# AKASH2907/pi-consistency-activity-detection

Hardware: AMD Instinct MI355X
Metric: train clips/sec (bs=8, 16×224×224, I3D+caps+bv cons) at 1/2/4/8 GPU (higher is better)
Workload: dtype f32 (fp32 operands and fp32 accumulation everywhere; 33 of the 79 conv / input-gradient launches and the 3x3x3 / 1x1x1 weight gradients multiply on the bf16 matrix cores: every fp32 operand as the exact sum of 3 bf16 terms, 6 products on v_mfma_f32_32x32x16_bf16, hi / lo fp32 accumulators -- error v

## Files before the change

### include/picons.h

```cpp
#ifndef PICONS_H
#define PICONS_H
#include <stdint.h>
#ifdef __cplusplus
extern "C" {
#endif

typedef void* pc_stream;

#define PC_OK            0
#define PC_E_ARG        -1
#define PC_E_LAUNCH     -2
#define PC_E_NODEVICE   -3

#define PC_ACT_NONE 0
#define PC_ACT_RELU 1
#define PC_ACT_SIGMOID 2

#define PC_F_ACCUM   1
#define PC_F_BIAS    2
#define PC_F_CSCALE  4
#define PC_F_BNPART  8
#define PC_F_NFAST   16
#define PC_F_TOUT    32
#define PC_F_CI3     64
// ... 109 lines not shown
int pc_bn_eval_stat(const float* gamma, const float* beta, const float* running_mean,
                    const float* running_var, float eps, int C, float* stat, pc_stream s);
int64_t pc_bn_bwd_ws_floats(int64_t rows, int C, int groups);
int pc_bn_bwd(const float* dy, int lddy, const float* z, int ldz, const float* stat, int C,
              int64_t rows, int groups, int relu, float* dz, int lddz, float* dgamma, float* dbeta,
              int accum, float* ws, pc_stream s);

typedef struct pc_pool_desc {
    int32_t N, Ti, Hi, Wi, C, ldi;
    int32_t To, Ho, Wo, ldo;
    int32_t k[3], s[3], padf[3];
} pc_pool_desc;
int pc_maxpool_fwd(const pc_pool_desc* d, const float* x, float* y, uint8_t* argmax, pc_stream s);
int pc_maxpool_bwd(const pc_pool_desc* d, const float* dy, const uint8_t* argmax, float* dx,
                   int accum, pc_stream s);

int pc_channel_scale(const float* x, int ldx, const float* scale, int N, int64_t pos_per_n, int C,
                     float* y, int ldy, int accum, pc_stream s);
int64_t pc_act_bwd_ws_floats(int64_t rows, int C);
int pc_act_bwd(const float* dy, int lddy, const float* y, int ldy, int act, int C, int64_t rows,
               float* dz, int lddz, float* dbias, int accum, float* ws, pc_stream s);
int pc_ncdhw_to_ndhwc(const void* src, int src_is_f64, int N, int C, int64_t thw, int W, int Cpad,
                      int flipw, float* dst, pc_stream s);
int pc_ndhwc_to_ncdhw(const float* src, int ld, int N, int C, int64_t thw, float* dst, pc_stream s);
int pc_transpose_batched(const float* src, int batch, int R, int Cc, int64_t src_batch_stride,
                         int src_ld, float* dst, int64_t dst_batch_stride, int dst_ld, int accum,
                         pc_stream s);
typedef struct pc_transpose_job {
    uint64_t src, dst;
    int64_t  src_batch_stride, dst_batch_stride;
// ... 208 lines not shown
```

### pi-consistency-activity-detection_amd/capi.py

```python
import ctypes as C
import os

import numpy as np

_HERE = os.path.dirname(os.path.abspath(__file__))
DIAG = os.environ.get("PICONS_DIAG_LIB", "0") not in ("", "0")
DIAG_SWITCHES = ("PICONS_CONV_ABLATE", "PICONS_WGRAD_ABLATE", "PICONS_WINO_VARIANT")
LIB_PATH = os.path.join(_HERE, "libpicons_diag.so" if DIAG else "libpicons.so")
if os.environ.get("PICONS_LIB_NAME"):
    LIB_PATH = os.path.join(_HERE, os.path.basename(os.environ["PICONS_LIB_NAME"]))
_lib = None

i32, i64, f32, vp = C.c_int32, C.c_int64, C.c_float, C.c_void_p


class ConvDesc(C.Structure):
    _fields_ = [(n, i32) for n in ("N", "Ti", "Hi", "Wi", "Ci", "ldi", "Tq", "Hq", "Wq", "To", "Ho", "Wo", "Co", "ldo")] + \
               [(n, i32 * 3) for n in ("ostr", "ooff", "istr", "ntap", "ioff0", "istep", "wk0", "wkstep")] + \
               [(n, i32) for n in ("KT", "KH", "KW", "ldw", "act", "flags", "wgstride", "bgstride", "act_c0", "groups")]


class WgradDesc(C.Structure):
    _fields_ = [(n, i32) for n in ("N", "Tq", "Hq", "Wq", "Cd", "ldd", "Ts", "Hs", "Ws", "Cs", "lds")] + \
               [(n, i32 * 3) for n in ("istr", "ntap", "ioff0", "istep", "wk0")] + [(n, i32) for n in ("KT", "KH", "KW", "splitk", "nbatch", "dbstride", "sbstride", "gbstride", "Td", "Hd", "Wd")] + [("doff", i32 * 3), ("flags", i32), ("ws_slices", i32)]
# ... 16 lines not shown


class LossDesc(C.Structure):
    _fields_ = [(n, i32) for n in ("B", "T", "H", "W", "bv", "gv", "n_frames", "predict_maps", "jhmdb")] + \
               [(n, f32) for n in ("lower_thresh", "upper_thresh", "bv_wt", "gv_wt", "wt_loc", "wt_cons", "wt_ramp")]


OP_DTYPE = np.dtype([("kind", np.int32), ("i", np.int32, 48), ("f", np.float32, 8), ("lane", np.int32),
                     ("p", np.uint64, 12), ("l", np.int64, 4)], align=False)

(OP_CONV, OP_WGRAD, OP_BN_FINALIZE, OP_BN_APPLY, OP_BN_EVAL_STAT, OP_BN_BWD, OP_POOL_FWD, OP_POOL_BWD, OP_CHSCALE,
 OP_ACT_BWD, OP_TO_NDHWC, OP_TO_NCDHW, OP_TRANSPOSE, OP_FILL, OP_AXPY, OP_EM_FWD, OP_EM_BWD, OP_CMASK_FWD, OP_CMASK_BWD,
 OP_TAPSUM_FWD, OP_TAPSUM_BWD, OP_LOSS, OP_SPREAD, OP_ADAM, OP_TAIL_COMBINE, OP_TAIL_COLSUM, OP_TAIL_GRADS, OP_COL2IM,
 OP_AXIS, OP_WSPEC_FWD, OP_WSPEC_BWD, OP_WSPEC_MASTER_FWD, OP_WSPEC_MASTER_BWD, OP_TAIL6_WEIGHTS, OP_TAIL6_GATHER, OP_TAIL6_SCATTER, OP_TAIL6_WGRAD_MAP, OP_TAIL6_BIAS_SUMS,
 OP_TRANSPOSE_MULTI, OP_FORK, OP_JOIN, OP_WGRAD_MULTI, OP_WINO_CONV, OP_WINO_WEIGHTS, OP_CONV_X6, OP_SPLIT_PLANES, OP_SPLIT_PLANES_MULTI, OP_WSPEC_MASTER_PLANES, OP_BN_FIN_APPLY, OP_WGRAD_FOLD, OP_WINO_WEIGHTS_MULTI, OP_VAL_METRICS) = range(1, 53)
MAX_LANES = 8

WJOB_DTYPE = np.dtype([("d", np.int32, 42), ("D", np.uint64), ("S", np.uint64), ("g", np.uint64)], align=False)

TJOB_DTYPE = np.dtype([("src", np.uint64), ("dst", np.uint64), ("sbs", np.int64), ("dbs", np.int64), ("batch", np.int32), ("R", np.int32),
                       ("C", np.int32), ("sld", np.int32), ("dld", np.int32), ("accum", np.int32), ("nslices", np.int32), ("reserved", np.int32),
                       ("sst", np.int64)], align=False)

SJOB_DTYPE = np.dtype([("src", np.uint64), ("planes", np.uint64), ("n", np.int64), ("pstride", np.int64)], align=False)

WWJOB_DTYPE = np.dtype([("w", np.uint64), ("U", np.uint64), ("sO", np.int64), ("sT", np.int64), ("sI", np.int64), ("O", np.int32), ("I", np.int32),
                        ("KT", np.int32), ("flip", np.int32), ("m", np.int32), ("reserved", np.int32)], align=False)

ACT_NONE, ACT_RELU, ACT_SIGMOID = 0, 1, 2
F_ACCUM, F_BIAS, F_CSCALE, F_BNPART, F_NFAST, F_TOUT, F_CI3, F_X6, F_STRIPS = 1, 2, 4, 8, 16, 32, 64, 128, 256
# ... 31 lines not shown
    "pc_wino4_u_floats": (i64, [i32, i32, i32]),
    "pc_wino4_weights": (i32, [vp, i64, i64, i64, i32, i32, i32, i32, vp, vp]),
    "pc_wino_bnpart_rows": (i32, [C.POINTER(WinoDesc)]),
    "pc_wino_work": (i32, [C.POINTER(WinoDesc), C.POINTER(C.c_double)]),
    "pc_bn_finalize": (i32, [vp, i32, i32, i32, i64, vp, vp, f32, f32, vp, vp, vp, vp]),
    "pc_bn_finalize_ws": (i32, [vp, i32, i32, i32, i64, vp, vp, f32, f32, vp, vp, vp, vp, vp]),
    "pc_bn_finalize_ws_floats": (i64, [i32, i32, i32]),
    "pc_bn_finalize_apply_ok": (i32, [i32, i32]),
    "pc_bn_finalize_apply": (i32, [vp, i32, i32, i32, i64, vp, vp, f32, f32, vp, vp, vp, vp, i32, i64, vp, i32, i32, vp]),
    "pc_bn_apply": (i32, [vp, i32, vp, i32, i64, i32, vp, i32, i32, vp]),
    "pc_bn_eval_stat": (i32, [vp, vp, vp, vp, f32, i32, vp, vp]),
    "pc_bn_bwd_ws_floats": (i64, [i64, i32, i32]),
    "pc_bn_bwd": (i32, [vp, i32, vp, i32, vp, i32, i64, i32, i32, vp, i32, vp, vp, i32, vp, vp]),
    "pc_maxpool_fwd": (i32, [C.POINTER(PoolDesc), vp, vp, vp, vp]),
    "pc_maxpool_bwd": (i32, [C.POINTER(PoolDesc), vp, vp, vp, i32, vp]),
    "pc_channel_scale": (i32, [vp, i32, vp, i32, i64, i32, vp, i32, i32, vp]),
    "pc_act_bwd_ws_floats": (i64, [i64, i32]),
    "pc_act_bwd": (i32, [vp, i32, vp, i32, i32, i32, i64, vp, i32, vp, i32, vp, vp]),
    "pc_ncdhw_to_ndhwc": (i32, [vp, i32, i32, i32, i64, i32, i32, i32, vp, vp]),
    "pc_ndhwc_to_ncdhw": (i32, [vp, i32, i32, i32, i64, vp, vp]),
    "pc_transpose_batched": (i32, [vp, i32, i32, i32, i64, i32, vp, i64, i32, i32, vp]),
    "pc_col2im": (i32, [vp, i32, i32, i32, i32, i32, i32, vp, i32, i32, vp]),
    "pc_seg_frame_counts": (i32, [vp, vp, i64, i64, vp, vp]),
    "pc_map_accumulate": (i32, [vp, i64, i32, i32, vp, vp, vp, vp, vp]),
    "pc_val_record_words": (i32, [i32]),
    "pc_val_metrics_ws_floats": (i64, [i32, i64]),
    "pc_val_metrics": (i32, [vp, vp, vp, vp, i32, i64, i32, vp, vp, vp]),
    "pc_clip_from_u8": (i32, [vp, i32, i32, i32, C.POINTER(C.c_int32), i32, i32, i32, vp, i32, vp, vp, vp, vp]),
    "pc_clip_from_u8_ndhwc4": (i32, [vp, i32, i32, i32, C.POINTER(C.c_int32), i32, i32, i32, vp, i32, vp, vp, vp, vp]),
    "pc_clip_from_u8_masks": (i32, [vp, i32, i32, i32, C.POINTER(C.c_int32), i32, i32, i32, vp, C.POINTER(C.c_int32), vp, vp, vp, vp, vp]),
# ... 122 lines not shown
```

### pi-consistency-activity-detection_amd/csrc/api.hip

```cpp
#include "common.h"
#include <string.h>
#include <vector>

static thread_local char g_err[512] = "";

void pc_set_error(const char* fmt, ...) {
    va_list ap;
    va_start(ap, fmt);
    vsnprintf(g_err, sizeof(g_err), fmt, ap);
    va_end(ap);
}

extern "C" const char* pc_last_error(void) { return g_err; }
extern "C" int pc_version(void) { return PC_VERSION; }

extern "C" int pc_transpose_batched(const float*, int, int, int, int64_t, int, float*, int64_t, int, int, pc_stream);

#define P(T, k) ((T)(uintptr_t)op.p[k])

static int run_one(const pc_op& op, pc_stream s) {
    switch (op.kind) {
        case PC_OP_CONV: {
            pc_conv_desc d;
            memcpy(&d, op.i, sizeof(d));
// ... 8 lines not shown
            return pc_split_planes(P(const float*, 0), P(uint16_t*, 1), op.l[0], op.l[1], s);
        case PC_OP_WSPEC_MASTER_PLANES:
            return pc_wspec_master_planes(P(const float*, 0), P(const float*, 1), op.i[0], op.i[1], op.i[2], op.i[3], op.i[4], op.i[5], op.i[6], op.i[7],
                                          P(uint16_t*, 2), P(uint16_t*, 3), op.l[0], s);
        case PC_OP_SPLIT_PLANES_MULTI:
            return pc_split_planes_multi(P(const pc_split_job*, 0), op.i[0], s);
        case PC_OP_WGRAD: {
            pc_wgrad_desc d;
            memcpy(&d, op.i, sizeof(d));
            return pc_conv_wgrad(&d, P(const float*, 0), P(const float*, 1), P(float*, 2), s);
        }
        case PC_OP_BN_FINALIZE:
            return pc_bn_finalize_ws(P(const float*, 0), op.i[0], op.i[1], op.i[2], op.l[0], P(const float*, 1), P(const float*, 2), op.f[0], op.f[1],
                                     P(float*, 3), P(float*, 4), P(float*, 5), P(float*, 6), s);
        case PC_OP_BN_APPLY:
            return pc_bn_apply(P(const float*, 0), op.i[0], P(const float*, 1), op.i[1], op.l[0], op.i[2], P(float*, 2), op.i[3], op.i[4], s);
        case PC_OP_BN_FIN_APPLY:
            return pc_bn_finalize_apply(P(const float*, 0), op.i[0], op.i[1], op.i[2], op.l[0], P(const float*, 1), P(const float*, 2), op.f[0], op.f[1], P(float*, 3),
                                        P(float*, 4), P(float*, 5), P(const float*, 6), op.i[3], op.l[1], P(float*, 7), op.i[4], op.i[5], s);
        case PC_OP_BN_EVAL_STAT:
            return pc_bn_eval_stat(P(const float*, 0), P(const float*, 1), P(const float*, 2), P(const float*, 3), op.f[0], op.i[0], P(float*, 4), s);
        case PC_OP_BN_BWD:
            return pc_bn_bwd(P(const float*, 0), op.i[0], P(const float*, 1), op.i[1], P(const float*, 2), op.i[2], op.l[0], op.i[3], op.i[4],
                             P(float*, 3), op.i[5], P(float*, 4), P(float*, 5), op.i[6], P(float*, 6), s);
        case PC_OP_POOL_FWD: {
            pc_pool_desc d;
            memcpy(&d, op.i, sizeof(d));
            return pc_maxpool_fwd(&d, P(const float*, 0), P(float*, 1), P(uint8_t*, 2), s);
        }
        case PC_OP_POOL_BWD: {
            pc_pool_desc d;
            memcpy(&d, op.i, sizeof(d));
            return pc_maxpool_bwd(&d, P(const float*, 0), P(const uint8_t*, 1), P(float*, 2), op.i[19], s);
        }
        case PC_OP_CHSCALE:
            return pc_channel_scale(P(const float*, 0), op.i[0], P(const float*, 1), op.i[1], op.l[0], op.i[2], P(float*, 2), op.i[3], op.i[4], s);
        case PC_OP_ACT_BWD:
// ... 260 lines not shown
```

### pi-consistency-activity-detection_amd/csrc/elementwise.hip

```cpp
#include "common.h"
#include <stdlib.h>

namespace {

constexpr int FIN_RL = 16;
constexpr int FIN_CL = 16;
constexpr int FIN_T = FIN_RL * FIN_CL;

template <typename TP>
__device__ __forceinline__ void partial_colsum(const TP* __restrict__ part, int npg, int C, int c, int rl,
                                               double (*sh)[FIN_RL][FIN_CL], int cl, double& s, double& s2) {
    double a[4] = {0, 0, 0, 0}, b[4] = {0, 0, 0, 0};
    if (c < C) {
        int i = rl;
        for (; i + 3 * FIN_RL < npg; i += 4 * FIN_RL) {
            TP x[4], y[4];
#pragma unroll
            for (int u = 0; u < 4; ++u) { const TP* q = part + (size_t)(i + u * FIN_RL) * 2 * C + c; x[u] = q[0]; y[u] = q[C]; }
#pragma unroll
            for (int u = 0; u < 4; ++u) { a[u] += (double)x[u]; b[u] += (double)y[u]; }
        }
        for (; i < npg; i += FIN_RL) { const TP* q = part + (size_t)i * 2 * C + c; a[0] += (double)q[0]; b[0] += (double)q[C]; }
    }
    sh[0][rl][cl] = (a[0] + a[1]) + (a[2] + a[3]); sh[1][rl][cl] = (b[0] + b[1]) + (b[2] + b[3]);
// ... 543 lines not shown
                        const int tap = (ho <= hi[1] && wo <= hi[2]) ? (a * KH + (h + d.padf[1] - ho * SH)) * KW + (w + d.padf[2] - wo * SW) : 256;
                        const uchar4 q = ix[jh * MW + jw];
                        const f32x4 u = v[jh * MW + jw];
                        if (q.x == tap) g[0] += u[0];
                        if (q.y == tap) g[1] += u[1];
                        if (q.z == tap) g[2] += u[2];
                        if (q.w == tap) g[3] += u[3];
                    }
            }
        }
        if (accum) g += old;
        *(f32x4*)o = g;
    }
}

constexpr int POOL_WT = 4;

template <int ST>
__global__ __launch_bounds__(256, 4) void maxpool333_fwd_tile_kernel(const pc_pool_desc d, const float* __restrict__ x, float* __restrict__ y,
                                                                     uint8_t* __restrict__ am, unsigned nitems) {
    const unsigned C4 = (unsigned)d.C / 4, tw = ((unsigned)d.Wo + 1) / 2, th = ((unsigned)d.Ho + 1) / 2;
    const unsigned i = (unsigned)xcd_remap((int)blockIdx.x, (int)gridDim.x) * 256 + threadIdx.x;
    if (i < nitems) {
        unsigned q = i / C4;
        const int c = (int)(i % C4) * 4;
        const int wo0 = (int)(q % tw) * 2; q /= tw;
        const int ho0 = (int)(q % th) * 2; q /= th;
        const int to = (int)(q % (unsigned)d.To); const int n = (int)(q / (unsigned)d.To);
        f32x4 best[4];
        unsigned bi[4];
// ... 544 lines not shown
#define PC_POOL_BWD_TILE(ST)                                                                                                                     \
    do {                                                                                                                                         \
        const int64_t items = pool_tile_items((int64_t)d->N * d->Ti * d->Hi, d->Wi, d->C / 4);                                                  \
        hipLaunchKernelGGL((maxpool333_bwd_tile_kernel<ST, POOL_WT>), dim3(items > 256 ? (unsigned)cdiv(items, 256) : 1), dim3(256), 0, (hipStream_t)s, \
                           *d, dy, argmax, dx, accum, (unsigned)items);                                                                          \
    } while (0)
    switch (pool_form(d)) {
        case 1: PC_POOL_BWD(1, 3, 3, 1, 2, 2); break;
        case 2: PC_POOL_BWD_TILE(2); break;
        case 3: PC_POOL_BWD_TILE(1); break;
        default: PC_POOL_BWD(0, 0, 0, 0, 0, 0);
    }
#undef PC_POOL_BWD_TILE
#undef PC_POOL_BWD
    PC_CHECK_LAUNCH("maxpool_bwd");
    return PC_OK;
}

extern "C" int pc_channel_scale(const float* x, int ldx, const float* scale, int N, int64_t pos_per_n, int C, float* y, int ldy,
                                int accum, pc_stream s) {
    PC_CHECK_ARG(x && scale && y && C % 4 == 0 && ldx % 4 == 0 && ldy % 4 == 0, "pc_channel_scale: bad args");
    const int64_t total4 = (int64_t)N * pos_per_n * (C / 4);
    PC_CHECK_ARG(total4 < (1ll << 31), "elementwise kernels index with 32 bits: %lld float4 elements", (long long)total4);
    hipLaunchKernelGGL(chscale_kernel, dim3(grid_for(total4, 2)), dim3(256), 0, (hipStream_t)s, x, ldx, scale, pos_per_n, C / 4, total4, y, ldy, accum);
    PC_CHECK_LAUNCH("channel_scale");
    return PC_OK;
}

extern "C" int64_t pc_act_bwd_ws_floats(int64_t rows, int C) {
    const int64_t rpb = red_rows_per_block(rows);
// ... 173 lines not shown
```

### pi-consistency-activity-detection_amd/ops.py

```python
import ctypes as C

import numpy as np
import torch

from . import capi, desc as D


def stream():
    return C.c_void_p(torch.cuda.current_stream().cuda_stream)


def ptr(t):
    if t is None:
        return None
    if not t.is_cuda:
        raise RuntimeError("picons ops need CUDA/HIP tensors (no CPU fallback)")
    return C.c_void_p(t.data_ptr())


def _fill_struct(st, d):
    for name, ctype in st._fields_:
        v = d[name]
        if isinstance(v, (list, tuple)):
            setattr(st, name, (C.c_int32 * 3)(*[int(x) for x in v]))
# ... 145 lines not shown


def bn_bwd(dy, lddy, z, ldz, stat, C_, rows, groups, relu, dz, lddz, dgamma, dbeta, accum=False, fused=False):
    ws = torch.empty(capi.lib().pc_bn_bwd_ws_floats(int(rows), C_, groups), device=dy.device, dtype=torch.float32)
    capi.call("pc_bn_bwd", ptr(dy), lddy, ptr(z), ldz, ptr(stat), C_, int(rows), groups, int(bool(relu)) | (2 if fused else 0), ptr(dz), lddz, ptr(dgamma), ptr(dbeta),
              int(accum), ptr(ws), stream())
    return dz


def maxpool_fwd(d, x, y, argmax):
    capi.call("pc_maxpool_fwd", C.byref(_fill_struct(capi.PoolDesc(), d)), ptr(x), ptr(y), ptr(argmax), stream())


def maxpool_bwd(d, dy, argmax, dx, accum=False):
    capi.call("pc_maxpool_bwd", C.byref(_fill_struct(capi.PoolDesc(), d)), ptr(dy), ptr(argmax), ptr(dx), int(accum), stream())


def channel_scale(x, ldx, scale, N, pos_per_n, C_, y, ldy, accum=False):
    capi.call("pc_channel_scale", ptr(x), ldx, ptr(scale), N, int(pos_per_n), C_, ptr(y), ldy, int(accum), stream())


def act_bwd(dy, lddy, y, ldy, act, C_, rows, dz, lddz, dbias=None, accum=False):
    ws = torch.empty(capi.lib().pc_act_bwd_ws_floats(int(rows), C_), device=dy.device, dtype=torch.float32)
    capi.call("pc_act_bwd", ptr(dy), lddy, ptr(y), ldy, act, C_, int(rows), ptr(dz), lddz, ptr(dbias), int(accum), ptr(ws), stream())


def to_ndhwc(src, Cpad=None, flipw=False):
    N, Cc, T, H, W = src.shape
    Cpad = Cpad or Cc
    dst = torch.empty(N, T, H, W, Cpad, device=src.device, dtype=torch.float32)
# ... 827 lines not shown
```

### pi-consistency-activity-detection_amd/plan.py

```python
from dataclasses import dataclass, field

import os

import numpy as np

from . import capi, desc as D, spec, spectral, switches as sw, tail6

ALIGN = 256


@dataclass
class TR:
    ref: tuple
    N: int
    thw: tuple
    C: int
    ld: int
    name: str = ""

    @property
    def rows(self):
        return self.N * self.thw[0] * self.thw[1] * self.thw[2]

    def slice(self, c0, c):
# ... 461 lines not shown
    def wgrad_group_end(self):
        jobs, self.wgrad_collect = self.wgrad_collect, None
        if not jobs:
            return

        def emit_all():
            if len(jobs) == 1 or self.wg_ordered or sw.exp("PICONS_WGRAD_MULTI", "0", self.exp) == "0":
                for d, p in jobs:
                    self._emit_wgrad(d, p)
            else:
                self.wjobs = getattr(self, "wjobs", [])
                self.wjobs.append(jobs)
                self.emit(capi.OP_WGRAD_MULTI, i=[len(jobs)], p=[("WJOBS", len(self.wjobs) - 1)])
        self.on_wgrad_lane(emit_all)

    def unit3d(self, pre, x, cout, k, stride, out=None, need_dx=True):
        pres, couts = ([pre], [cout]) if isinstance(pre, str) else (list(pre), list(cout))
        pre, cout = pres[0], sum(couts)
        for tab, sfxs in ((self.poff, (".bn.weight", ".bn.bias")), (self.roff, (".bn.running_mean", ".bn.running_var"))):
            for sfx in sfxs:
                o = tab[pre + sfx]
                for q, c in zip(pres, couts):
                    if tab[q + sfx] != o:
                        raise RuntimeError("stacked Unit3Ds need adjacent %s (%s)" % (sfx, q))
                    o += c
        Ci = x.C
        Ci_real = self.pshape[pre + ".conv3d.weight"][1]
        othw = tuple(spec.same_out(x.thw[i], k[i], stride[i]) for i in range(3))
        pf = [spec.same_pad(x.thw[i], k[i], stride[i])[0] for i in range(3)]
        wino = len(pres) == 1 and Ci == Ci_real and self.wino_ok(x, cout, k, stride)
        w = self.prep_conv_weight([q + ".conv3d.weight" for q in pres], couts, Ci_real, k, need_dx, Ipad=Ci, layouts=not wino)
# ... 28 lines not shown
            trunk_x6 = sw.exp("PICONS_SPLIT_TRUNK_FWD", "0", self.exp) != "0"
            if trunk_x6:
                d = self.maybe_x6(d, w["fwd"])
            nrows = _bnpart_rows(d)
            part = self.alloc(nrows * 2 * cout)
            self.conv_op(d, x.ref, w["fwd"], z.ref, bnpart=part, x6=trunk_x6)
            fin = self.bn_finalize_or_defer(nrows, cout, z, part, gamma, beta, pre, stat)
            g_apply = self.groups
        else:
            d = D.conv_fwd(x.N, x.thw, Ci, x.ld, cout, z.ld, k, stride, pf, othw, flags=capi.F_CI3 if ci3 else 0)
            d["Ci_real"] = Ci_real
            self.conv_op(d, x.ref, w["fwd"], z.ref)
            self.emit(capi.OP_BN_EVAL_STAT, i=[cout], f=[spec.BN_EPS],
                      p=[gamma, beta, self.R(pre + ".bn.running_mean"), self.R(pre + ".bn.running_var"), stat])
            g_apply = 1
        if fin is not None:
            self.emit(capi.OP_BN_FIN_APPLY, i=[fin["npg"], self.groups, cout, z.ld, y.ld, 1], l=[z.rows // self.groups, z.rows], f=[spec.BN_EPS, spec.BN_MOMENTUM],
                      p=[fin["part"], gamma, beta, self.R(pre + ".bn.running_mean"), self.R(pre + ".bn.running_var"), stat, z.ref, y.ref])
        else:
            self.emit(capi.OP_BN_APPLY, i=[z.ld, cout, g_apply, y.ld, 1], l=[z.rows], p=[z.ref, stat, y.ref])

        st = {}

        def bwd(part="all"):
            if part in ("all", "A"):
                dy = self.grad_of(y)
                dz = st["dz"] = self.tensor(x.N, othw, cout, pre + ".dz")
                ws = self.alloc(_bn_bwd_ws(z.rows, cout, self.groups))
                fused_bwd = 2 if sw.exp("PICONS_BN_FUSED", "0", self.exp) != "0" else 0
                self.emit(capi.OP_BN_BWD, i=[dy.ld, z.ld, cout, self.groups, 1 | fused_bwd, dz.ld, self.acc], l=[z.rows],
                          p=[dy.ref, z.ref, stat, dz.ref, self.G(pre + ".bn.weight"), self.G(pre + ".bn.bias"), ws])
                if self.after_bn_bwd is not None:
                    hook, self.after_bn_bwd = self.after_bn_bwd, None
                    hook()
                wd = D.trim_wgrad(D.wgrad(x.N, othw, cout, dz.ld, x.thw, Ci, x.ld, k, stride, pf))
                wd["Cs_real"] = Ci_real
                wd["flags"] = capi.WG_CS3 if ci3 else 0
                self.on_wgrad_lane(lambda: (self.wgrad_op(wd, [dz.ref, x.ref, w["kg"]], w), self.flush_grad(w)))
                self.mark_final(*[q + sfx for q in pres for sfx in (".bn.weight", ".bn.bias")])
            if need_dx and part in ("all", "B"):
                dz = st["dz"]
                dx, acc = self.grad_for_write(x)
                self.alg_dgrad(F_fwd, wino)
                if wino:
                    self.wino_op(dz.ref, x.N, x.thw, othw[0], cout, dz.ld, Ci, dx.ld, tmap_b, wu["tr"], dx.ref, flags=capi.F_ACCUM if acc else 0, m=wm_b)
                else:
# ... 263 lines not shown
        self.in_drop128 = self.alloc(N * 128)
        x = self.tensor(N, (T, hw, hw), 4, "img")
        self.img = x
        self.op_to_ndhwc = []
        for g in range(self.groups):
            self.op_to_ndhwc.append(len(self.lists["fwd"]))
            src = self.in_data if g == 0 else self.in_aug
            self.emit(capi.OP_TO_NDHWC, i=[0, self.n, 3, hw, 4, 0], l=[T * hw * hw], p=[src, off(x.ref, g * self.n * T * hw * hw * 4)])
        out56 = out112 = None
        first = True
        s28e = hw // 8
        if self.skip_lane:
            cat56 = self.tensor(N, (2, 2 * s28e, 2 * s28e), 128, "cat56")
            cat112 = self.tensor(N, (4, 4 * s28e, 4 * s28e), 128, "cat112")
        pending_skip, skip_after = [], sw.exp("PICONS_SKIP_FWD_AFTER", "", self.exp)
        for ent in spec.TRUNK:
            name = "conv1." + ent[0]
            if ent[0] == "Mixed_3b" and self.late_prep:
                self.join(1 << self.wg_lane)
            if ent[1] == "conv":
                x = self.unit3d(name, x, ent[3], ent[4], ent[5], need_dx=not first)
                first = False
            elif ent[1] == "pool":
                x = self.maxpool(x, ent[2], ent[3], name)
            else:
                x = self.inception(name, x, ent[3])
            if ent[0] == "Conv3d_2c_3x3":
                out56 = x
                if self.skip_lane:
                    pending_skip.append(("conv56", out56, cat56))
            if ent[0] == "Conv3d_1a_7x7":
                out112 = x
                if self.skip_lane:
                    pending_skip.append(("conv112", out112, cat112))
            if pending_skip and (not skip_after or ent[0] == skip_after or ent is spec.TRUNK[-1]):
                for nm_, t_, c_ in pending_skip:
                    self._skip_conv(nm_, t_, c_)
                pending_skip = []
            if ent[0] == "MaxPool3d_3a_3x3" and self.skip_lane:
                inner = self.tape.pop()
                self.tape.append(lambda inner=inner: (self.join(1 << self.skip_lane), inner()))
        self.named["trunk_out"] = x
        s28 = x.thw[1]
        if self.training:
            xd = self.tensor(N, x.thw, x.C, "x832d")
            self.emit(capi.OP_CHSCALE, i=[x.ld, N, x.C, xd.ld, 0], l=[x.rows // N], p=[x.ref, self.in_drop832, xd.ref])
            xin = x

            def bwd_drop():
                dxd = self.grad_of(xd)
                dx, acc = self.grad_for_write(xin)
                self.emit(capi.OP_CHSCALE, i=[dxd.ld, N, xin.C, dx.ld, int(acc)], l=[xin.rows // N], p=[dxd.ref, self.in_drop832, dx.ref])
            self.tape.append(bwd_drop)
        else:
            xd = x
        cat28 = self.tensor(N, (1, s28, s28), 128, "cat28")
# ... 585 lines not shown
```

Baseline: 454.3.

## Fuse BN apply with following (1,3,3)/(1,2,2) maxpool in forward and backward

When a conv unit is immediately followed by a 1x3x3 stride 1x2x2 SAME maxpool, the BN-apply kernel now also computes the pooled output and argmax, and BN backward reads the pooled gradient and argmax directly instead of a separate maxpool-backward pass writing dy. This removes the standalone pool forward and backward kernels and one full read/write of the pre-pool activation gradient. In exchange the fused kernels re-read overlapping z windows, BN finalize becomes a separate launch, and the backward reduce recomputes the pool scatter per row.

```diff
diff --git a/include/picons.h b/include/picons.h
--- a/include/picons.h
+++ b/include/picons.h
@@ -147,6 +147,11 @@
 int pc_maxpool_fwd(const pc_pool_desc* d, const float* x, float* y, uint8_t* argmax, pc_stream s);
 int pc_maxpool_bwd(const pc_pool_desc* d, const float* dy, const uint8_t* argmax, float* dx,
                    int accum, pc_stream s);
+int pc_bn_apply_pool(const pc_pool_desc* d, const float* z, int ldz, const float* stat, int groups, int relu, float* y, float* yp,
+                     uint8_t* argmax, pc_stream s);
+int pc_bn_bwd_pool(const pc_pool_desc* d, const float* base, const float* dyp, const uint8_t* argmax, const float* z, int ldz,
+                   const float* stat, int groups, int relu, float* dz, int lddz, float* dgamma, float* dbeta, int accum, float* ws,
+                   pc_stream s);
 
 int pc_channel_scale(const float* x, int ldx, const float* scale, int N, int64_t pos_per_n, int C,
                      float* y, int ldy, int accum, pc_stream s);
diff --git a/pi-consistency-activity-detection_amd/capi.py b/pi-consistency-activity-detection_amd/capi.py
--- a/pi-consistency-activity-detection_amd/capi.py
+++ b/pi-consistency-activity-detection_amd/capi.py
@@ -54,6 +54,14 @@
  OP_TAPSUM_FWD, OP_TAPSUM_BWD, OP_LOSS, OP_SPREAD, OP_ADAM, OP_TAIL_COMBINE, OP_TAIL_COLSUM, OP_TAIL_GRADS, OP_COL2IM,
  OP_AXIS, OP_WSPEC_FWD, OP_WSPEC_BWD, OP_WSPEC_MASTER_FWD, OP_WSPEC_MASTER_BWD, OP_TAIL6_WEIGHTS, OP_TAIL6_GATHER, OP_TAIL6_SCATTER, OP_TAIL6_WGRAD_MAP, OP_TAIL6_BIAS_SUMS,
  OP_TRANSPOSE_MULTI, OP_FORK, OP_JOIN, OP_WGRAD_MULTI, OP_WINO_CONV, OP_WINO_WEIGHTS, OP_CONV_X6, OP_SPLIT_PLANES, OP_SPLIT_PLANES_MULTI, OP_WSPEC_MASTER_PLANES, OP_BN_FIN_APPLY, OP_WGRAD_FOLD, OP_WINO_WEIGHTS_MULTI, OP_VAL_METRICS) = range(1, 53)
+BN_POOL_AT = 8
+
+
+def bn_pool_ints(kind, ints):
+    flag = {OP_BN_APPLY: 5, OP_BN_BWD: 7}.get(kind)
+    if flag is None or len(ints) <= BN_POOL_AT or not ints[flag]:
+        return None
+    return [int(v) for v in ints[BN_POOL_AT:BN_POOL_AT + 19]]
 MAX_LANES = 8
 
 WJOB_DTYPE = np.dtype([("d", np.int32, 42), ("D", np.uint64), ("S", np.uint64), ("g", np.uint64)], align=False)
@@ -115,6 +123,8 @@
     "pc_bn_bwd": (i32, [vp, i32, vp, i32, vp, i32, i64, i32, i32, vp, i32, vp, vp, i32, vp, vp]),
     "pc_maxpool_fwd": (i32, [C.POINTER(PoolDesc), vp, vp, vp, vp]),
     "pc_maxpool_bwd": (i32, [C.POINTER(PoolDesc), vp, vp, vp, i32, vp]),
+    "pc_bn_apply_pool": (i32, [C.POINTER(PoolDesc), vp, i32, vp, i32, i32, vp, vp, vp, vp]),
+    "pc_bn_bwd_pool": (i32, [C.POINTER(PoolDesc), vp, vp, vp, vp, i32, vp, i32, i32, vp, i32, vp, vp, i32, vp, vp]),
     "pc_channel_scale": (i32, [vp, i32, vp, i32, i64, i32, vp, i32, i32, vp]),
     "pc_act_bwd_ws_floats": (i64, [i64, i32]),
     "pc_act_bwd": (i32, [vp, i32, vp, i32, i32, i32, i64, vp, i32, vp, i32, vp, vp]),
diff --git a/pi-consistency-activity-detection_amd/csrc/api.hip b/pi-consistency-activity-detection_amd/csrc/api.hip
--- a/pi-consistency-activity-detection_amd/csrc/api.hip
+++ b/pi-consistency-activity-detection_amd/csrc/api.hip
@@ -46,6 +46,12 @@
             return pc_bn_finalize_ws(P(const float*, 0), op.i[0], op.i[1], op.i[2], op.l[0], P(const float*, 1), P(const float*, 2), op.f[0], op.f[1],
                                      P(float*, 3), P(float*, 4), P(float*, 5), P(float*, 6), s);
         case PC_OP_BN_APPLY:
+            if (op.i[5]) {
+                pc_pool_desc d;
+                memcpy(&d, op.i + 8, sizeof(d));
+                if (d.C != op.i[1] || d.ldi != op.i[3] || (int64_t)d.N * d.Ti * d.Hi * d.Wi != op.l[0]) { pc_set_error("PC_OP_BN_APPLY: pool descriptor and unit disagree"); return PC_E_ARG; }
+                return pc_bn_apply_pool(&d, P(const float*, 0), op.i[0], P(const float*, 1), op.i[2], op.i[4], P(float*, 2), P(float*, 3), P(uint8_t*, 4), s);
+            }
             return pc_bn_apply(P(const float*, 0), op.i[0], P(const float*, 1), op.i[1], op.l[0], op.i[2], P(float*, 2), op.i[3], op.i[4], s);
         case PC_OP_BN_FIN_APPLY:
             return pc_bn_finalize_apply(P(const float*, 0), op.i[0], op.i[1], op.i[2], op.l[0], P(const float*, 1), P(const float*, 2), op.f[0], op.f[1], P(float*, 3),
@@ -53,6 +59,13 @@
         case PC_OP_BN_EVAL_STAT:
             return pc_bn_eval_stat(P(const float*, 0), P(const float*, 1), P(const float*, 2), P(const float*, 3), op.f[0], op.i[0], P(float*, 4), s);
         case PC_OP_BN_BWD:
+            if (op.i[7]) {
+                pc_pool_desc d;
+                memcpy(&d, op.i + 8, sizeof(d));
+                if (d.C != op.i[2] || d.ldi != op.i[0] || (int64_t)d.N * d.Ti * d.Hi * d.Wi != op.l[0]) { pc_set_error("PC_OP_BN_BWD: pool descriptor and unit disagree"); return PC_E_ARG; }
+                return pc_bn_bwd_pool(&d, P(const float*, 0), P(const float*, 7), P(const uint8_t*, 8), P(const float*, 1), op.i[1], P(const float*, 2), op.i[3],
+                                      op.i[4], P(float*, 3), op.i[5], P(float*, 4), P(float*, 5), op.i[6], P(float*, 6), s);
+            }
             return pc_bn_bwd(P(const float*, 0), op.i[0], P(const float*, 1), op.i[1], P(const float*, 2), op.i[2], op.l[0], op.i[3], op.i[4],
                              P(float*, 3), op.i[5], P(float*, 4), P(float*, 5), op.i[6], P(float*, 6), s);
         case PC_OP_POOL_FWD: {
diff --git a/pi-consistency-activity-detection_amd/csrc/elementwise.hip b/pi-consistency-activity-detection_amd/csrc/elementwise.hip
--- a/pi-consistency-activity-detection_amd/csrc/elementwise.hip
+++ b/pi-consistency-activity-detection_amd/csrc/elementwise.hip
@@ -581,6 +581,241 @@
     }
 }
 
+__global__ __launch_bounds__(256) void bn_apply_pool_kernel(const pc_pool_desc d, const float* __restrict__ z, int ldz, const float* __restrict__ stat,
+                                                            int n_per_group, int relu, float* __restrict__ y, float* __restrict__ yp,
+                                                            uint8_t* __restrict__ am, unsigned npos, unsigned ppb) {
+    const unsigned C4 = (unsigned)d.C / 4;
+    const unsigned p0 = (unsigned)xcd_remap((int)blockIdx.x, (int)gridDim.x) * ppb;
+    if (p0 >= npos) return;
+    const unsigned items = (min(npos, p0 + ppb) - p0) * C4;
+    for (unsigned i = threadIdx.x; i < items; i += 256) {
+        unsigned pos = p0 + i / C4;
+        const int c = (int)(i % C4) * 4;
+        const size_t opos = pos;
+        const int wo = (int)(pos % (unsigned)d.Wo); pos /= (unsigned)d.Wo;
+        const int ho = (int)(pos % (unsigned)d.Ho); pos /= (unsigned)d.Ho;
+        const int t = (int)(pos % (unsigned)d.To); const int n = (int)(pos / (unsigned)d.To);
+        const float* st = stat + (size_t)(n / n_per_group) * 4 * d.C;
+        const f32x4 sc = *(const f32x4*)(st + 2 * d.C + c), sh = *(const f32x4*)(st + 3 * d.C + c);
+        const int h0 = ho * 2 - d.padf[1], w0 = wo * 2 - d.padf[2];
+        const size_t frame = (size_t)(n * d.Ti + t) * d.Hi * d.Wi;
+        f32x4 v[9];
+#pragma unroll
+        for (int b = 0; b < 3; ++b)
+#pragma unroll
+            for (int cc = 0; cc < 3; ++cc) {
+                const int h = min(max(h0 + b, 0), d.Hi - 1), w = min(max(w0 + cc, 0), d.Wi - 1);
+                v[b * 3 + cc] = *(const f32x4*)(z + (frame + (size_t)h * d.Wi + w) * ldz + c);
+            }
+        f32x4 best = {-INFINITY, -INFINITY, -INFINITY, -INFINITY};
+        int bi[4] = {255, 255, 255, 255};
+#pragma unroll
+        for (int b = 0; b < 3; ++b)
+#pragma unroll
+            for (int cc = 0; cc < 3; ++cc) {
+                const bool inb = (unsigned)(h0 + b) < (unsigned)d.Hi && (unsigned)(w0 + cc) < (unsigned)d.Wi;
+                f32x4 o;
+#pragma unroll
+                for (int e = 0; e < 4; ++e) { const float q = v[b * 3 + cc][e] * sc[e] + sh[e]; o[e] = relu ? fmaxf(q, 0.f) : q; }
+                if (inb && (b < 2 || ho == d.Ho - 1) && (cc < 2 || wo == d.Wo - 1))
+                    *(f32x4*)(y + (frame + (size_t)(h0 + b) * d.Wi + (w0 + cc)) * d.ldi + c) = o;
+                const int tap = b * 3 + cc;
+#pragma unroll
+                for (int e = 0; e < 4; ++e) {
+                    const float u = inb ? o[e] : 0.f;
+                    if (u > best[e]) { best[e] = u; bi[e] = inb ? tap : 255; }
+                }
+            }
+        *(f32x4*)(yp + opos * d.ldo + c) = best;
+        *(uchar4*)(am + opos * d.C + c) = make_uchar4(bi[0], bi[1], bi[2], bi[3]);
+    }
+}
+
+__device__ __forceinline__ f32x4 pool122_dy(const pc_pool_desc& d, const float* __restrict__ dyp, const uint8_t* __restrict__ am,
+                                            const float* __restrict__ base, unsigned ipos, unsigned frame, int h, int w, int c) {
+    f32x4 old = {0.f, 0.f, 0.f, 0.f};
+    if (base) old = *(const f32x4*)(base + (size_t)ipos * d.ldi + c);
+    f32x4 g = {0.f, 0.f, 0.f, 0.f};
+    int lo[2], hi[2];
+    const int xs[2] = {h, w}, Os[2] = {d.Ho, d.Wo};
+#pragma unroll
+    for (int q = 0; q < 2; ++q) {
+        const int top = xs[q] + d.padf[1 + q], bot = top - 3 + 1;
+        hi[q] = min(top / 2, Os[q] - 1);
+        lo[q] = bot <= 0 ? 0 : (bot + 2 - 1) / 2;
+    }
+    uchar4 ix[4];
+    f32x4 v[4];
+#pragma unroll
+    for (int jh = 0; jh < 2; ++jh)
+#pragma unroll
+        for (int jw = 0; jw < 2; ++jw) {
+            const int ho = lo[0] + jh, wo = lo[1] + jw;
+            ix[jh * 2 + jw] = make_uchar4(255, 255, 255, 255);
+            v[jh * 2 + jw] = f32x4{0.f, 0.f, 0.f, 0.f};
+            if (ho <= hi[0] && wo <= hi[1]) {
+                const size_t op = ((size_t)frame * d.Ho + ho) * d.Wo + wo;
+                ix[jh * 2 + jw] = *(const uchar4*)(am + op * d.C + c);
+                v[jh * 2 + jw] = *(const f32x4*)(dyp + op * d.ldo + c);
+            }
+        }
+#pragma unroll
+    for (int jh = 0; jh < 2; ++jh)
+#pragma unroll
+        for (int jw = 0; jw < 2; ++jw) {
+            const int ho = lo[0] + jh, wo = lo[1] + jw;
+            const int tap = (ho <= hi[0] && wo <= hi[1]) ? (h + d.padf[1] - ho * 2) * 3 + (w + d.padf[2] - wo * 2) : 256;
+            const uchar4 q = ix[jh * 2 + jw];
+            const f32x4 u = v[jh * 2 + jw];
+            if (q.x == tap) g[0] += u[0];
+            if (q.y == tap) g[1] += u[1];
+            if (q.z == tap) g[2] += u[2];
+            if (q.w == tap) g[3] += u[3];
+        }
+    if (base) g += old;
+    return g;
+}
+
+struct RedPoolP {
+    pc_pool_desc d; const float* base; const float* dyp; const uint8_t* am;
+    const float* z; int ldz; const float* stat; int64_t rows_per_group, rows_per_block; int relu; float* part; int npg;
+};
+
+__global__ __launch_bounds__(256) void colreduce_pool_kernel(RedPoolP p) {
+    const int C = p.d.C, C4 = C / 4;
+    const int rpi = 256 / C4;
+    const int c4 = threadIdx.x % C4, rl = threadIdx.x / C4;
+    const bool active = rl < rpi;
+    const int blk = xcd_remap((int)blockIdx.x, (int)gridDim.x);
+    const int64_t g0 = (int64_t)blockIdx.y * p.rows_per_group;
+    const int64_t r0 = (int64_t)blk * p.rows_per_block;
+    const int64_t r1 = min(p.rows_per_group, r0 + p.rows_per_block);
+    const float* st = p.stat + (size_t)blockIdx.y * 4 * C;
+    double sd[8] = {0, 0, 0, 0, 0, 0, 0, 0};
+    if (active) {
+        const int c = c4 * 4;
+        float s[8] = {0, 0, 0, 0, 0, 0, 0, 0};
+        int run = 0;
+        const f32x4 mean = *(const f32x4*)(st + c), inv = *(const f32x4*)(st + C + c);
+        const f32x4 sc = *(const f32x4*)(st + 2 * C + c), sh_ = *(const f32x4*)(st + 3 * C + c);
+        unsigned pos = (unsigned)(g0 + r0 + rl);
+        int w = (int)(pos % (unsigned)p.d.Wi); pos /= (unsigned)p.d.Wi;
+        int h = (int)(pos % (unsigned)p.d.Hi);
+        unsigned frame = pos / (unsigned)p.d.Hi;
+        for (int64_t r = r0 + rl; r < r1; r += rpi) {
+            const f32x4 zz = *(const f32x4*)(p.z + (g0 + r) * p.ldz + c);
+            const f32x4 dy = pool122_dy(p.d, p.dyp, p.am, p.base, (unsigned)(g0 + r), frame, h, w, c);
+            w += rpi;
+            while (w >= p.d.Wi) { w -= p.d.Wi; if (++h == p.d.Hi) { h = 0; ++frame; } }
+#pragma unroll
+            for (int e = 0; e < 4; ++e) {
+                const float yv = zz[e] * sc[e] + sh_[e];
+                const float d = (p.relu && !(yv > 0.f)) ? 0.f : dy[e];
+                s[e] += d;
+                s[4 + e] += d * (zz[e] - mean[e]) * inv[e];
+            }
+            if (++run == 4) {
+                run = 0;
+#pragma unroll
+                for (int e = 0; e < 8; ++e) { sd[e] += (double)s[e]; s[e] = 0.f; }
+            }
+        }
+#pragma unroll
+        for (int e = 0; e < 8; ++e) sd[e] += (double)s[e];
+    }
+    __shared__ double shd[256 * 8];
+#pragma unroll
+    for (int e = 0; e < 8; ++e) shd[threadIdx.x * 8 + e] = sd[e];
+    __syncthreads();
+    if (threadIdx.x < C4) {
+        double t[8] = {0, 0, 0, 0, 0, 0, 0, 0};
+        for (int q = 0; q < rpi; ++q)
+#pragma unroll
+            for (int e = 0; e < 8; ++e) t[e] += shd[(q * C4 + threadIdx.x) * 8 + e];
+        float* o = p.part + ((size_t)blockIdx.y * p.npg + blk) * 2 * C + threadIdx.x * 4;
+#pragma unroll
+        for (int e = 0; e < 4; ++e) { o[e] = (float)t[e]; o[C + e] = (float)t[4 + e]; }
+    }
+}
+
+__global__ __launch_bounds__(256) void bn_bwd_apply_pool_kernel(const pc_pool_desc d, const float* __restrict__ base, const float* __restrict__ dyp,
+                                                                const uint8_t* __restrict__ am, const float* __restrict__ z, int ldz,
+                                                                const float* __restrict__ stat, const float* __restrict__ coef,
+                                                                unsigned frames_per_group, int relu, float* __restrict__ dz, int lddz,
+                                                                unsigned ntile, unsigned tpb) {
+    const unsigned C4 = (unsigned)d.C / 4;
+    const int C = d.C;
+    const unsigned Bh = (unsigned)(d.Hi + d.padf[1] + 1) / 2, Bw = (unsigned)(d.Wi + d.padf[2] + 1) / 2;
+    const unsigned p0 = (unsigned)xcd_remap((int)blockIdx.x, (int)gridDim.x) * tpb;
+    if (p0 >= ntile) return;
+    const unsigned items = (min(ntile, p0 + tpb) - p0) * C4;
+    for (unsigned i = threadIdx.x; i < items; i += 256) {
+        unsigned q = p0 + i / C4;
+        const int c = (int)(i % C4) * 4;
+        const int n_ = (int)(q % Bw); q /= Bw;
+        const int m = (int)(q % Bh);
+        const unsigned frame = q / Bh;
+        const int g = (int)(frame / frames_per_group);
+        const float* st = stat + (size_t)g * 4 * C;
+        const float* cf = coef + (size_t)g * 2 * C;
+        uchar4 ix[4];
+        f32x4 v[4], old[4], zz[4];
+#pragma unroll
+        for (int jh = 0; jh < 2; ++jh)
+#pragma unroll
+            for (int jw = 0; jw < 2; ++jw) {
+                const int ho = min(max(m - 1 + jh, 0), d.Ho - 1), wo = min(max(n_ - 1 + jw, 0), d.Wo - 1);
+                const size_t op = ((size_t)frame * d.Ho + ho) * d.Wo + wo;
+                ix[jh * 2 + jw] = *(const uchar4*)(am + op * d.C + c);
+                v[jh * 2 + jw] = *(const f32x4*)(dyp + op * d.ldo + c);
+            }
+#pragma unroll
+        for (int a = 0; a < 2; ++a)
+#pragma unroll
+            for (int b = 0; b < 2; ++b) {
+                const int h = min(max(2 * m + a - d.padf[1], 0), d.Hi - 1), w = min(max(2 * n_ + b - d.padf[2], 0), d.Wi - 1);
+                const size_t row = ((size_t)frame * d.Hi + h) * d.Wi + w;
+                old[a * 2 + b] = f32x4{0.f, 0.f, 0.f, 0.f};
+                if (base) old[a * 2 + b] = *(const f32x4*)(base + row * d.ldi + c);
+                zz[a * 2 + b] = *(const f32x4*)(z + row * ldz + c);
+            }
+        const f32x4 mean = *(const f32x4*)(st + c), inv = *(const f32x4*)(st + C + c);
+        const f32x4 sc = *(const f32x4*)(st + 2 * C + c), sh_ = *(const f32x4*)(st + 3 * C + c);
+        const f32x4 c1 = *(const f32x4*)(cf + c), c2 = *(const f32x4*)(cf + C + c);
+#pragma unroll
+        for (int a = 0; a < 2; ++a)
+#pragma unroll
+            for (int b = 0; b < 2; ++b) {
+                const int h = 2 * m + a - d.padf[1], w = 2 * n_ + b - d.padf[2];
+                if ((unsigned)h >= (unsigned)d.Hi || (unsigned)w >= (unsigned)d.Wi) continue;
+                f32x4 gsum = {0.f, 0.f, 0.f, 0.f};
+#pragma unroll
+                for (int jh = a; jh < 2; ++jh)
+#pragma unroll
+                    for (int jw = b; jw < 2; ++jw) {
+                        const bool inw = (unsigned)(m - 1 + jh) < (unsigned)d.Ho && (unsigned)(n_ - 1 + jw) < (unsigned)d.Wo;
+                        const int tap = inw ? (a + 2 - 2 * jh) * 3 + (b + 2 - 2 * jw) : 256;
+                        const uchar4 k = ix[jh * 2 + jw];
+                        const f32x4 u = v[jh * 2 + jw];
+                        if (k.x == tap) gsum[0] += u[0];
+                        if (k.y == tap) gsum[1] += u[1];
+                        if (k.z == tap) gsum[2] += u[2];
+                        if (k.w == tap) gsum[3] += u[3];
+                    }
+                if (base) gsum += old[a * 2 + b];
+                const f32x4 zv = zz[a * 2 + b];
+                f32x4 o;
+#pragma unroll
+                for (int e = 0; e < 4; ++e) {
+                    const float yv = zv[e] * sc[e] + sh_[e];
+                    const float dd = (relu && !(yv > 0.f)) ? 0.f : gsum[e];
+                    o[e] = sc[e] * (dd - c1[e] - (zv[e] - mean[e]) * inv[e] * c2[e]);
+                }
+                *(f32x4*)(dz + (((size_t)frame * d.Hi + h) * d.Wi + w) * lddz + c) = o;
+            }
+    }
+}
+
 constexpr int POOL_WT = 4;
 
 template <int ST>
@@ -1155,6 +1390,56 @@
 #undef PC_POOL_BWD_TILE
 #undef PC_POOL_BWD
     PC_CHECK_LAUNCH("maxpool_bwd");
+    return PC_OK;
+}
+
+static bool pool122_ok(const pc_pool_desc* d) {
+    return pool_form(d) == 1 && d->To == d->Ti && d->padf[0] == 0 && d->Ho >= 1 && d->Wo >= 1 &&
+           (d->padf[1] == 0 || d->padf[1] == 1) && (d->padf[2] == 0 || d->padf[2] == 1) &&
+           2 * d->Ho - d->padf[1] >= d->Hi - 1 && 2 * d->Wo - d->padf[2] >= d->Wi - 1 && 2 * (d->Ho - 1) - d->padf[1] < d->Hi && 2 * (d->Wo - 1) - d->padf[2] < d->Wi;
+}
+
+extern "C" int pc_bn_apply_pool(const pc_pool_desc* d, const float* z, int ldz, const float* stat, int groups, int relu, float* y, float* yp,
+                                uint8_t* argmax, pc_stream s) {
+    PC_CHECK_ARG(d && z && stat && y && yp && argmax && d->C > 0 && d->C % 4 == 0 && ldz % 4 == 0 && d->ldi % 4 == 0 && d->ldo % 4 == 0 && ldz >= d->C &&
+                 d->ldi >= d->C && d->ldo >= d->C && groups >= 1 && d->N >= 1 && d->N % groups == 0, "pc_bn_apply_pool: bad args");
+    PC_CHECK_ARG(pool122_ok(d), "pc_bn_apply_pool: the (1,3,3)/(1,2,2) SAME pool only");
+    const int64_t npos = (int64_t)d->N * d->To * d->Ho * d->Wo, total4 = npos * (d->C / 4);
+    PC_CHECK_ARG((int64_t)d->N * d->Ti * d->Hi * d->Wi * (d->C / 4) < (1ll << 31), "elementwise kernels index with 32 bits");
+    const int nblk = pool_blocks(total4);
+    const unsigned ppb = (unsigned)cdiv(npos, nblk);
+    hipLaunchKernelGGL(bn_apply_pool_kernel, dim3(nblk), dim3(256), 0, (hipStream_t)s, *d, z, ldz, stat, d->N / groups, relu, y, yp, argmax, (unsigned)npos, ppb);
+    PC_CHECK_LAUNCH("bn_apply_pool");
+    return PC_OK;
+}
+
+extern "C" int pc_bn_bwd_pool(const pc_pool_desc* d, const float* base, const float* dyp, const uint8_t* argmax, const float* z, int ldz,
+                              const float* stat, int groups, int relu, float* dz, int lddz, float* dgamma, float* dbeta, int accum, float* ws,
+                              pc_stream s_) {
+    hipStream_t s = (hipStream_t)s_;
+    PC_CHECK_ARG(d && dyp && argmax && z && stat && dz && ws && d->C > 0 && d->C % 4 == 0 && d->C <= 1024 && d->ldi % 4 == 0 && d->ldo % 4 == 0 && ldz % 4 == 0 &&
+                 lddz % 4 == 0 && d->ldi >= d->C && d->ldo >= d->C && ldz >= d->C && lddz >= d->C && groups >= 1 && d->N >= 1 && d->N % groups == 0,
+                 "pc_bn_bwd_pool: bad args");
+    PC_CHECK_ARG(pool122_ok(d), "pc_bn_bwd_pool: the (1,3,3)/(1,2,2) SAME pool only");
+    const int C = d->C;
+    const int64_t rows = (int64_t)d->N * d->Ti * d->Hi * d->Wi, rpg = rows / groups, total4 = rows * (C / 4);
+    PC_CHECK_ARG(total4 < (1ll << 31), "elementwise kernels index with 32 bits: %lld float4 elements", (long long)total4);
+    const int64_t rpb = red_rows_per_block(rpg);
+    const int npg = (int)((rpg + rpb - 1) / rpb);
+    float* part = ws;
+    float* coef = ws + (size_t)npg * groups * 2 * C;
+    RedPoolP p;
+    p.d = *d; p.base = base; p.dyp = dyp; p.am = argmax; p.z = z; p.ldz = ldz; p.stat = stat;
+    p.rows_per_group = rpg; p.rows_per_block = rpb; p.relu = relu & 1; p.part = part; p.npg = npg;
+    hipLaunchKernelGGL(colreduce_pool_kernel, dim3(npg, groups), dim3(256), 0, s, p);
+    PC_CHECK_LAUNCH("bn_bwd_pool reduce");
+    hipLaunchKernelGGL(bn_bwd_finalize_kernel, dim3(cdiv(C, FIN_CL)), dim3(FIN_T), 0, s, part, npg, groups, C, (double)rpg, coef, dgamma, dbeta, accum);
+    const int64_t ntile = (int64_t)d->N * d->Ti * ((d->Hi + d->padf[1] + 1) / 2) * ((d->Wi + d->padf[2] + 1) / 2);
+    const int nblk = pool_blocks(ntile * (C / 4));
+    const unsigned tpb = (unsigned)cdiv(ntile, nblk);
+    hipLaunchKernelGGL(bn_bwd_apply_pool_kernel, dim3(nblk), dim3(256), 0, s, *d, base, dyp, argmax, z, ldz, stat, coef, (unsigned)(d->N / groups * d->Ti),
+                       relu & 1, dz, lddz, (unsigned)ntile, tpb);
+    PC_CHECK_LAUNCH("bn_bwd_pool apply");
     return PC_OK;
 }
 
diff --git a/pi-consistency-activity-detection_amd/ops.py b/pi-consistency-activity-detection_amd/ops.py
--- a/pi-consistency-activity-detection_amd/ops.py
+++ b/pi-consistency-activity-detection_amd/ops.py
@@ -183,6 +183,18 @@
 
 def maxpool_bwd(d, dy, argmax, dx, accum=False):
     capi.call("pc_maxpool_bwd", C.byref(_fill_struct(capi.PoolDesc(), d)), ptr(dy), ptr(argmax), ptr(dx), int(accum), stream())
+
+
+def bn_apply_pool(d, z, ldz, stat, groups, y, yp, argmax, relu=True):
+    capi.call("pc_bn_apply_pool", C.byref(_fill_struct(capi.PoolDesc(), d)), ptr(z), ldz, ptr(stat), groups, int(relu), ptr(y), ptr(yp), ptr(argmax), stream())
+
+
+def bn_bwd_pool(d, base, dyp, argmax, z, ldz, stat, groups, relu, dz, lddz, dgamma, dbeta, accum=False):
+    rows = d["N"] * d["Ti"] * d["Hi"] * d["Wi"]
+    ws = torch.empty(capi.lib().pc_bn_bwd_ws_floats(int(rows), d["C"], groups), device=z.device, dtype=torch.float32)
+    capi.call("pc_bn_bwd_pool", C.byref(_fill_struct(capi.PoolDesc(), d)), ptr(base), ptr(dyp), ptr(argmax), ptr(z), ldz, ptr(stat), groups, int(bool(relu)),
+              ptr(dz), lddz, ptr(dgamma), ptr(dbeta), int(accum), ptr(ws), stream())
+    return dz
 
 
 def channel_scale(x, ldx, scale, N, pos_per_n, C_, y, ldy, accum=False):
diff --git a/pi-consistency-activity-detection_amd/plan.py b/pi-consistency-activity-detection_amd/plan.py
--- a/pi-consistency-activity-detection_amd/plan.py
+++ b/pi-consistency-activity-detection_amd/plan.py
@@ -499,7 +499,7 @@
                 self.emit(capi.OP_WGRAD_MULTI, i=[len(jobs)], p=[("WJOBS", len(self.wjobs) - 1)])
         self.on_wgrad_lane(emit_all)
 
-    def unit3d(self, pre, x, cout, k, stride, out=None, need_dx=True):
+    def unit3d(self, pre, x, cout, k, stride, out=None, need_dx=True, pool=None):
         pres, couts = ([pre], [cout]) if isinstance(pre, str) else (list(pre), list(cout))
         pre, cout = pres[0], sum(couts)
         for tab, sfxs in ((self.poff, (".bn.weight", ".bn.bias")), (self.roff, (".bn.running_mean", ".bn.running_var"))):
@@ -558,7 +558,21 @@
             self.emit(capi.OP_BN_EVAL_STAT, i=[cout], f=[spec.BN_EPS],
                       p=[gamma, beta, self.R(pre + ".bn.running_mean"), self.R(pre + ".bn.running_var"), stat])
             g_apply = 1
-        if fin is not None:
+        pl = None
+        if pool is not None:
+            if fin is not None:
+                self.emit(capi.OP_BN_FINALIZE, i=[fin["npg"], self.groups, cout], l=[z.rows // self.groups], f=[spec.BN_EPS, spec.BN_MOMENTUM],
+                          p=[fin["part"], gamma, beta, self.R(pre + ".bn.running_mean"), self.R(pre + ".bn.running_var"), stat, self.bn_fin_ws(fin["npg"], cout)])
+            pk, ps, pname = pool
+            pthw = tuple(spec.same_out(othw[i], pk[i], ps[i]) for i in range(3))
+            ppad = [spec.same_pad(othw[i], pk[i], ps[i])[0] for i in range(3)]
+            yp = self.tensor(x.N, pthw, cout, pname)
+            am = self.alloc((yp.rows * cout + 3) // 4)
+            pl = dict(yp=yp, am=am, thw=pthw, k=pk, s=ps, padf=ppad)
+            self.pooled = yp
+            pd = D.flatten(D.pool(x.N, othw, cout, y.ld, pthw, yp.ld, pk, ps, ppad), D.POOL_FIELDS)
+            self.emit(capi.OP_BN_APPLY, i=[z.ld, cout, g_apply, y.ld, 1, 1, 0, 0] + pd, l=[z.rows], p=[z.ref, stat, y.ref, yp.ref, am])
+        elif fin is not None:
             self.emit(capi.OP_BN_FIN_APPLY, i=[fin["npg"], self.groups, cout, z.ld, y.ld, 1], l=[z.rows // self.groups, z.rows], f=[spec.BN_EPS, spec.BN_MOMENTUM],
                       p=[fin["part"], gamma, beta, self.R(pre + ".bn.running_mean"), self.R(pre + ".bn.running_var"), stat, z.ref, y.ref])
         else:
@@ -567,13 +581,22 @@
         st = {}
 
         def bwd(part="all"):
-            if part in ("all", "A"):
+            if part in ("all", "A") and pl is not None:
+                dyp = self.grad_of(pl["yp"])
+                base = self.grad_of(y) if (y.name in self.grads and self.grads[y.name][1]) else None
+                dz = st["dz"] = self.tensor(x.N, othw, cout, pre + ".dz")
+                ws = self.alloc(_bn_bwd_ws(z.rows, cout, self.groups))
+                pdb = D.flatten(D.pool(x.N, othw, cout, base.ld if base is not None else y.ld, pl["thw"], dyp.ld, pl["k"], pl["s"], pl["padf"]), D.POOL_FIELDS)
+                self.emit(capi.OP_BN_BWD, i=[pdb[5], z.ld, cout, self.groups, 1, dz.ld, self.acc, 1] + pdb, l=[z.rows],
+                          p=[base.ref if base is not None else None, z.ref, stat, dz.ref, self.G(pre + ".bn.weight"), self.G(pre + ".bn.bias"), ws, dyp.ref, pl["am"]])
+            elif part in ("all", "A"):
                 dy = self.grad_of(y)
                 dz = st["dz"] = self.tensor(x.N, othw, cout, pre + ".dz")
                 ws = self.alloc(_bn_bwd_ws(z.rows, cout, self.groups))
                 fused_bwd = 2 if sw.exp("PICONS_BN_FUSED", "0", self.exp) != "0" else 0
                 self.emit(capi.OP_BN_BWD, i=[dy.ld, z.ld, cout, self.groups, 1 | fused_bwd, dz.ld, self.acc], l=[z.rows],
                           p=[dy.ref, z.ref, stat, dz.ref, self.G(pre + ".bn.weight"), self.G(pre + ".bn.bias"), ws])
+            if part in ("all", "A"):
                 if self.after_bn_bwd is not None:
                     hook, self.after_bn_bwd = self.after_bn_bwd, None
                     hook()
@@ -867,13 +890,20 @@
             cat56 = self.tensor(N, (2, 2 * s28e, 2 * s28e), 128, "cat56")
             cat112 = self.tensor(N, (4, 4 * s28e, 4 * s28e), 128, "cat112")
         pending_skip, skip_after = [], sw.exp("PICONS_SKIP_FWD_AFTER", "", self.exp)
-        for ent in spec.TRUNK:
+        pool_in_bn = sw.get("PICONS_POOL_IN_BN", "1") != "0"
+        unit_y = None
+        for ei, ent in enumerate(spec.TRUNK):
             name = "conv1." + ent[0]
             if ent[0] == "Mixed_3b" and self.late_prep:
                 self.join(1 << self.wg_lane)
             if ent[1] == "conv":
-                x = self.unit3d(name, x, ent[3], ent[4], ent[5], need_dx=not first)
+                nxt = spec.TRUNK[ei + 1] if ei + 1 < len(spec.TRUNK) else None
+                ride = pool_in_bn and nxt is not None and nxt[1] == "pool" and tuple(nxt[2]) == (1, 3, 3) and tuple(nxt[3]) == (1, 2, 2)
+                x = self.unit3d(name, x, ent[3], ent[4], ent[5], need_dx=not first, pool=(nxt[2], nxt[3], "conv1." + nxt[0]) if ride else None)
+                unit_y = x if ride else None
                 first = False
+            elif ent[1] == "pool" and unit_y is not None:
+                x, unit_y = self.pooled, None
             elif ent[1] == "pool":
                 x = self.maxpool(x, ent[2], ent[3], name)
             else:
@@ -892,7 +922,7 @@
                 pending_skip = []
             if ent[0] == "MaxPool3d_3a_3x3" and self.skip_lane:
                 inner = self.tape.pop()
-                self.tape.append(lambda inner=inner: (self.join(1 << self.skip_lane), inner()))
+                self.tape.append(lambda *a, inner=inner: (self.join(1 << self.skip_lane), inner(*a)))
         self.named["trunk_out"] = x
         s28 = x.thw[1]
         if self.training:
```

Result: no change. 454.1, median of 4 (-0.0%).
